# octree-nn/octfusion

Hardware: AMD Instinct MI355X
Metric: denoising-steps/sec (depth-8 octree, batch 8) (higher is better)
Workload: dtype f32 storage, fp16x3 products (fp16 hi + lo operand pairs = 22 significand bits, three fp16 MFMAs per product, fp32 accumulate)

## Files before the change

octfusion_amd/csrc/ofx_dense.hip:

```cpp
#include "ofx_common.h"

__global__ void grid_table_kernel(int mode, int d_out, int B, int32_t pad, int32_t* __restrict__ nbr) {
  const int S = 1 << d_out;
  const int64_t per = (int64_t)S * S * S, total = per * B * 27;
  const int d_in = mode == 0 ? d_out : (mode == 1 ? d_out + 1 : d_out - 1);
  const int Sin = 1 << d_in;
  for (int64_t t = (int64_t)blockIdx.x * blockDim.x + threadIdx.x; t < total; t += (int64_t)gridDim.x * blockDim.x) {
    const int64_t row = t / 27;
    const int tap = (int)(t - row * 27);
    const int64_t b = row / per;
    int x, y, z, bb;
    ofx_key2xyz(row - b * per, x, y, z, bb);
    const int tx = tap / 9 - 1, ty = (tap / 3) % 3 - 1, tz = tap % 3 - 1;
    int ix, iy, iz;
    bool ok;
    if (mode == 0) {
      ix = x + tx; iy = y + ty; iz = z + tz;
      ok = ix >= 0 && iy >= 0 && iz >= 0 && ix < S && iy < S && iz < S;
    } else if (mode == 1) {
      ix = 2 * x + tx; iy = 2 * y + ty; iz = 2 * z + tz;
      ok = ix >= 0 && iy >= 0 && iz >= 0 && ix < Sin && iy < Sin && iz < Sin;
    } else {
      const int fx = x + tx, fy = y + ty, fz = z + tz;
      ok = fx >= 0 && fy >= 0 && fz >= 0 && fx < S && fy < S && fz < S;
      ix = fx >> 1; iy = fy >> 1; iz = fz >> 1;
    }
    nbr[t] = ok ? (int32_t)(b * ((int64_t)Sin * Sin * Sin) + (int64_t)ofx_xyz2morton(ix, iy, iz)) : pad;
  }
}

extern "C" int ofx_grid_conv_table(int mode, int depth_out, int batch_size, int32_t pad, int32_t* nbr27, void* stream) {
  if (mode < 0 || mode > 2 || depth_out < 0 || depth_out > 8 || batch_size < 1 || !nbr27) return OFX_EINVAL;
  if (mode == 2 && depth_out < 1) return OFX_EINVAL;
  const int64_t total = (1ll << (3 * depth_out)) * batch_size * 27;
  grid_table_kernel<<<ofx_grid(total, 256), 256, 0, ofx_stream(stream)>>>(mode, depth_out, batch_size, pad, nbr27);
  OFX_LAUNCH_CHECK();
  return OFX_OK;
}

typedef float f32x16d __attribute__((ext_vector_type(16)));

template <int CH, bool SPLIT>
__global__ void __launch_bounds__(256, 1) attention_mfma_kernel(const float* __restrict__ qkv, int64_t ldq, int T,
                                                                int heads, int ch, float* __restrict__ out,
                                                                int64_t ldo) {
  __shared__ float cmb[4][32][2];
  constexpr int KLD = CH + 4;
  extern __shared__ __attribute__((aligned(16))) float smem[];
  const int Tp = (T + 31) & ~31;
  float* Ks = smem;
  float* Vs = smem + (size_t)Tp * KLD;
  const int bh = blockIdx.x;
  const int b = bh / heads, hd = bh - b * heads;
  const int64_t row0 = (int64_t)b * T;
  const float scale = 1.f / sqrtf(sqrtf((float)ch));
  const int lane = threadIdx.x & 63, wid = threadIdx.x >> 6;
  const int l31 = lane & 31, h = lane >> 5;

  const float* kbase = qkv + row0 * ldq + (int64_t)hd * 3 * ch + ch;
  if ((ch & 3) == 0 && (ldq & 3) == 0 && (((uintptr_t)qkv) & 15) == 0) {
    constexpr int C4 = CH / 4;
    const int total = Tp * C4;
    for (int i0 = threadIdx.x; i0 < total; i0 += 4 * blockDim.x) {
      float4 kq[4], vq[4];
#pragma unroll
      for (int u = 0; u < 4; ++u) {
        const int i = i0 + u * blockDim.x;
        const int s = i / C4, c = (i - s * C4) * 4;
        kq[u] = make_float4(0.f, 0.f, 0.f, 0.f);
        vq[u] = kq[u];
        if (i < total && s < T && c < ch) {
          const float* p = kbase + (int64_t)s * ldq + c;
          kq[u] = *reinterpret_cast<const float4*>(p);
          vq[u] = *reinterpret_cast<const float4*>(p + ch);
        }
      }
#pragma unroll
      for (int u = 0; u < 4; ++u) {
        const int i = i0 + u * blockDim.x;
        if (i >= total) continue;
        const int s = i / C4, c = (i - s * C4) * 4;
        *reinterpret_cast<float4*>(Ks + s * KLD + c) = make_float4(kq[u].x * scale, kq[u].y * scale, kq[u].z * scale, kq[u].w * scale);
        *reinterpret_cast<float4*>(Vs + s * KLD + c) = vq[u];
      }
    }
  } else {
    for (int i = threadIdx.x; i < Tp * CH; i += blockDim.x) {
      const int s = i / CH, c = i - s * CH;
      float kv = 0.f, vv = 0.f;
      if (s < T && c < ch) {
        const float* p = kbase + (int64_t)s * ldq + c;
        kv = p[0] * scale;
        vv = p[ch];
      }
      Ks[s * KLD + c] = kv;
      Vs[s * KLD + c] = vv;
    }
  }
  __syncthreads();

  const int q0 = SPLIT ? blockIdx.y * 32 : blockIdx.y * 128 + wid * 32;
  if (q0 >= T) return;
  const int qi = q0 + l31;
  const bool qok = qi < T;
  float qreg[CH / 2];
  {
    const float* qp = qkv + (row0 + (qok ? qi : T - 1)) * ldq + (int64_t)hd * 3 * ch;
#pragma unroll
    for (int s = 0; s < CH / 2; ++s) {
      const int c = h * (CH / 2) + s;
      qreg[s] = (c < ch) ? qp[c] * scale : 0.f;
    }
  }
  const int ntile = Tp / 32;

  auto score_tile = [&](int kt, f32x16d& st) {
#pragma unroll
    for (int r = 0; r < 16; ++r) st[r] = 0.f;
    const float* kr = Ks + (kt * 32 + l31) * KLD + h * (CH / 2);
#pragma unroll
    for (int s4 = 0; s4 < CH / 8; ++s4) {
      const float4 kv = *reinterpret_cast<const float4*>(kr + s4 * 4);
      st = __builtin_amdgcn_mfma_f32_32x32x2f32(kv.x, qreg[s4 * 4 + 0], st, 0, 0, 0);
      st = __builtin_amdgcn_mfma_f32_32x32x2f32(kv.y, qreg[s4 * 4 + 1], st, 0, 0, 0);
      st = __builtin_amdgcn_mfma_f32_32x32x2f32(kv.z, qreg[s4 * 4 + 2], st, 0, 0, 0);
      st = __builtin_amdgcn_mfma_f32_32x32x2f32(kv.w, qreg[s4 * 4 + 3], st, 0, 0, 0);
    }
    if (kt * 32 + 32 > T) {
#pragma unroll
      for (int r = 0; r < 16; ++r)
        if (kt * 32 + (r & 3) + 8 * (r >> 2) + 4 * h >= T) st[r] = -INFINITY;
    }
  };

  const int kt0 = SPLIT ? (wid * ntile) / 4 : 0, kt1 = SPLIT ? ((wid + 1) * ntile) / 4 : ntile;

  float mx = -INFINITY, den = 0.f;
  for (int kt = kt0; kt < kt1; ++kt) {
    f32x16d st;
    score_tile(kt, st);
    float tm = st[0];
#pragma unroll
    for (int r = 1; r < 16; ++r) tm = fmaxf(tm, st[r]);
    tm = fmaxf(tm, __shfl_xor(tm, 32, 64));
    const float mn = fmaxf(mx, tm);
    float ps = 0.f;
#pragma unroll
    for (int r = 0; r < 16; ++r) ps += __expf(st[r] - mn);
    ps += __shfl_xor(ps, 32, 64);
    den = den * __expf(mx - mn) + ps;
    mx = mn;
  }
  if (SPLIT) {
    if (h == 0) { cmb[wid][l31][0] = mx; cmb[wid][l31][1] = den; }
    __syncthreads();
    float gm = -INFINITY;
#pragma unroll
    for (int w = 0; w < 4; ++w) gm = fmaxf(gm, cmb[w][l31][0]);
    float gd = 0.f;
#pragma unroll
    for (int w = 0; w < 4; ++w) {
      const float mw = cmb[w][l31][0];
      gd += mw == -INFINITY ? 0.f : cmb[w][l31][1] * __expf(mw - gm);
    }
    mx = gm; den = gd;
  }
  const float inv = 1.f / den;

  f32x16d oacc[CH / 32];
#pragma unroll
  for (int j = 0; j < CH / 32; ++j)
#pragma unroll
    for (int r = 0; r < 16; ++r) oacc[j][r] = 0.f;
  for (int kt = kt0; kt < kt1; ++kt) {
    f32x16d st;
    score_tile(kt, st);
#pragma unroll
    for (int r = 0; r < 16; ++r) st[r] = __expf(st[r] - mx) * inv;
    const float* vr = Vs + (kt * 32 + 4 * h) * KLD + l31;
#pragma unroll
    for (int r = 0; r < 16; ++r) {
      const float* vrow = vr + ((r & 3) + 8 * (r >> 2)) * KLD;
#pragma unroll
      for (int j = 0; j < CH / 32; ++j)
        oacc[j] = __builtin_amdgcn_mfma_f32_32x32x2f32(st[r], vrow[j * 32], oacc[j], 0, 0, 0);
    }
  }
  if (SPLIT) {
    __syncthreads();
    float* osum = Ks;
#pragma unroll
    for (int j = 0; j < CH / 32; ++j)
#pragma unroll
      for (int r = 0; r < 16; ++r)
        osum[(wid * 32 + (r & 3) + 8 * (r >> 2) + 4 * h) * CH + j * 32 + l31] = oacc[j][r];
    __syncthreads();
    for (int i = threadIdx.x; i < 32 * CH; i += 256) {
      const int q = i / CH, c = i - q * CH;
      if (q0 + q < T && c < ch)
        out[(row0 + q0 + q) * ldo + (int64_t)hd * ch + c] = (osum[i] + osum[32 * CH + i]) + (osum[64 * CH + i] + osum[96 * CH + i]);
    }
    return;
  }
#pragma unroll
  for (int j = 0; j < CH / 32; ++j) {
    const int c = j * 32 + l31;
    if (c >= ch) continue;
#pragma unroll
    for (int r = 0; r < 16; ++r) {
      const int q = q0 + (r & 3) + 8 * (r >> 2) + 4 * h;
      if (q < T) out[(row0 + q) * ldo + (int64_t)hd * ch + c] = oacc[j][r];
    }
  }
}

static int g_attn_split = 1;
extern "C" int ofx_set_attention_split(int on) { g_attn_split = on ? 1 : 0; return OFX_OK; }

template <int CH>
static int launch_attention(const float* qkv, int64_t ldq, int B, int T, int heads, int ch, float* out, int64_t ldo,
                            hipStream_t st) {
  const int Tp = (T + 31) & ~31;
  const size_t lds = (size_t)2 * Tp * (CH + 4) * sizeof(float);
  if (lds > 160 * 1024 - 2048) return OFX_EINVAL;
  static bool attr_set[OFX_MAX_DEVICES] = {}, attr_set_split[OFX_MAX_DEVICES] = {};
  if (T >= 256 && g_attn_split) {
    if (!ofx_raise_lds_limit(reinterpret_cast<const void*>(&attention_mfma_kernel<CH, true>), 160 * 1024 - 2048, attr_set_split))
      return OFX_ELAUNCH;
    dim3 grid((unsigned)(B * heads), (unsigned)ofx_cdiv(T, 32));
    attention_mfma_kernel<CH, true><<<grid, 256, lds, st>>>(qkv, ldq, T, heads, ch, out, ldo);
    return OFX_OK;
  }
  if (!ofx_raise_lds_limit(reinterpret_cast<const void*>(&attention_mfma_kernel<CH, false>), 160 * 1024 - 2048, attr_set))
    return OFX_ELAUNCH;
  dim3 grid((unsigned)(B * heads), (unsigned)ofx_cdiv(T, 128));
  attention_mfma_kernel<CH, false><<<grid, 256, lds, st>>>(qkv, ldq, T, heads, ch, out, ldo);
  return OFX_OK;
}

extern "C" int ofx_attention(const float* qkv, int64_t ldq, int batch_size, int T, int heads, int ch, float* out,
                             int64_t ldo, void* stream) {
  if (!qkv || !out || batch_size < 1 || T < 1 || heads < 1 || ch < 1 || ch > 128 || ldq < 3 * (int64_t)heads * ch ||
      ldo < (int64_t)heads * ch)
    return OFX_EINVAL;
  hipStream_t st = ofx_stream(stream);
  int rc;
  if (ch <= 32) rc = launch_attention<32>(qkv, ldq, batch_size, T, heads, ch, out, ldo, st);
  else if (ch <= 64) rc = launch_attention<64>(qkv, ldq, batch_size, T, heads, ch, out, ldo, st);
  else rc = launch_attention<128>(qkv, ldq, batch_size, T, heads, ch, out, ldo, st);
  if (rc) return rc;
  OFX_LAUNCH_CHECK();
  return OFX_OK;
}


__device__ __forceinline__ float score_rounded(float a, float sc) {
#pragma clang fp contract(off)
  return a * sc;
}
__device__ __forceinline__ float wave_sum(float v) {
#pragma unroll
  for (int o = 32; o > 0; o >>= 1) v += __shfl_xor(v, o);
  return v;
}
__device__ __forceinline__ float wave_max(float v) {
#pragma unroll
  for (int o = 32; o > 0; o >>= 1) v = fmaxf(v, __shfl_xor(v, o));
  return v;
}

__global__ void __launch_bounds__(256) attention_bwd_q_kernel(const float* __restrict__ qkv, int64_t ldq,
                                                              const float* __restrict__ dout, int64_t ldo, int T,
                                                              int heads, int ch, float* __restrict__ rowstat,
                                                              float* __restrict__ dqkv, int64_t ldd) {
  extern __shared__ float lds[];
  const int lane = threadIdx.x & 63, wid = threadIdx.x >> 6;
  const int bh = blockIdx.y, b = bh / heads, hd = bh - b * heads;
  const int i = blockIdx.x * 4 + wid;
  if (i >= T) return;
  float* ds = lds + wid * T;
  const float sc = rsqrtf((float)ch);
  const int64_t row0 = (int64_t)b * T;
  const float* qi = qkv + (row0 + i) * ldq + (int64_t)hd * 3 * ch;
  const float* gi = dout + (row0 + i) * ldo + (int64_t)hd * ch;
  const float* kb = qkv + row0 * ldq + (int64_t)hd * 3 * ch + ch;
  const float* vb = kb + ch;
  const bool vec = (ch & 3) == 0 && (ldq & 3) == 0 && (ldo & 3) == 0 && ((((uintptr_t)qkv) | ((uintptr_t)dout)) & 15) == 0;
  float s[8], dp[8];
  float m = -3.0e38f;
#pragma unroll
  for (int t = 0; t < 8; ++t) {
    const int j = lane + 64 * t;
    s[t] = -3.0e38f; dp[t] = 0.f;
    if (j < T) {
      float a = 0.f, d = 0.f;
      const float* kj = kb + (int64_t)j * ldq;
      const float* vj = vb + (int64_t)j * ldq;
      if (vec) {
        for (int c = 0; c < ch; c += 4) {
          const float4 q4 = *reinterpret_cast<const float4*>(qi + c), g4 = *reinterpret_cast<const float4*>(gi + c);
          const float4 k4 = *reinterpret_cast<const float4*>(kj + c), v4 = *reinterpret_cast<const float4*>(vj + c);
          a += q4.x * k4.x + q4.y * k4.y + q4.z * k4.z + q4.w * k4.w;
          d += g4.x * v4.x + g4.y * v4.y + g4.z * v4.z + g4.w * v4.w;
        }
      } else {
        for (int c = 0; c < ch; ++c) { a += qi[c] * kj[c]; d += gi[c] * vj[c]; }
      }
      s[t] = score_rounded(a, sc); dp[t] = d;
      m = fmaxf(m, s[t]);
    }
  }
  m = wave_max(m);
  float l = 0.f;
#pragma unroll
  for (int t = 0; t < 8; ++t) { const int j = lane + 64 * t; if (j < T) { s[t] = __expf(s[t] - m); l += s[t]; } }
  l = wave_sum(l);
  const float inv = 1.f / l;
  float D = 0.f;
#pragma unroll
  for (int t = 0; t < 8; ++t) { const int j = lane + 64 * t; if (j < T) { s[t] *= inv; D += s[t] * dp[t]; } }
  D = wave_sum(D);
#pragma unroll
  for (int t = 0; t < 8; ++t) { const int j = lane + 64 * t; if (j < T) ds[j] = s[t] * (dp[t] - D); }
  if (lane == 0) {
    float* rs = rowstat + ((int64_t)bh * T + i) * 3;
    rs[0] = m; rs[1] = inv; rs[2] = D;
  }
  __builtin_amdgcn_wave_barrier();
  for (int c = lane; c < ch; c += 64) {
    float a = 0.f;
    for (int j = 0; j < T; ++j) a += ds[j] * kb[(int64_t)j * ldq + c];
    dqkv[(row0 + i) * ldd + (int64_t)hd * 3 * ch + c] = a * sc;
  }
}

__global__ void __launch_bounds__(256) attention_bwd_kv_kernel(const float* __restrict__ qkv, int64_t ldq,
                                                               const float* __restrict__ dout, int64_t ldo, int T,
                                                               int heads, int ch, const float* __restrict__ rowstat,
                                                               float* __restrict__ dqkv, int64_t ldd) {
  extern __shared__ float lds[];
  const int lane = threadIdx.x & 63, wid = threadIdx.x >> 6;
  const int bh = blockIdx.y, b = bh / heads, hd = bh - b * heads;
  const int j = blockIdx.x * 4 + wid;
  if (j >= T) return;
  float* pc = lds + wid * 2 * T;
  float* dc = pc + T;
  const float sc = rsqrtf((float)ch);
  const int64_t row0 = (int64_t)b * T;
  const float* qb = qkv + row0 * ldq + (int64_t)hd * 3 * ch;
  const float* kj = qb + (int64_t)j * ldq + ch;
  const float* vj = kj + ch;
  const float* gb = dout + row0 * ldo + (int64_t)hd * ch;
  const float* rs = rowstat + (int64_t)bh * T * 3;
  const bool vec = (ch & 3) == 0 && (ldq & 3) == 0 && (ldo & 3) == 0 && ((((uintptr_t)qkv) | ((uintptr_t)dout)) & 15) == 0;
  for (int i = lane; i < T; i += 64) {
    float a = 0.f, d = 0.f;
    const float* qr = qb + (int64_t)i * ldq;
    const float* gr = gb + (int64_t)i * ldo;
    if (vec) {
      for (int c = 0; c < ch; c += 4) {
        const float4 q4 = *reinterpret_cast<const float4*>(qr + c), g4 = *reinterpret_cast<const float4*>(gr + c);
        const float4 k4 = *reinterpret_cast<const float4*>(kj + c), v4 = *reinterpret_cast<const float4*>(vj + c);
        a += q4.x * k4.x + q4.y * k4.y + q4.z * k4.z + q4.w * k4.w;
        d += g4.x * v4.x + g4.y * v4.y + g4.z * v4.z + g4.w * v4.w;
      }
    } else {
      for (int c = 0; c < ch; ++c) { a += qr[c] * kj[c]; d += gr[c] * vj[c]; }
    }
    const float p = __expf(score_rounded(a, sc) - rs[i * 3]) * rs[i * 3 + 1];
    pc[i] = p;
    dc[i] = p * (d - rs[i * 3 + 2]);
  }
  __builtin_amdgcn_wave_barrier();
  for (int c = lane; c < ch; c += 64) {
    float dk = 0.f, dv = 0.f;
    for (int i = 0; i < T; ++i) { dk += dc[i] * qb[(int64_t)i * ldq + c]; dv += pc[i] * gb[(int64_t)i * ldo + c]; }
    float* o = dqkv + (row0 + j) * ldd + (int64_t)hd * 3 * ch;
    o[ch + c] = dk * sc;
    o[2 * ch + c] = dv;
  }
}

extern "C" int ofx_attention_bwd(const float* qkv, int64_t ldq, const float* dout, int64_t ldo, int batch_size, int T,
                                 int heads, int ch, float* rowstat, float* dqkv, int64_t ldd, void* stream) {
  if (!qkv || !dout || !rowstat || !dqkv || batch_size < 1 || T < 1 || T > 512 || heads < 1 || ch < 1 ||
      ldq < 3 * (int64_t)heads * ch || ldd < 3 * (int64_t)heads * ch || ldo < (int64_t)heads * ch)
    return OFX_EINVAL;
  hipStream_t st = ofx_stream(stream);
  const dim3 grid((unsigned)((T + 3) / 4), (unsigned)(batch_size * heads));
  attention_bwd_q_kernel<<<grid, 256, 4 * T * sizeof(float), st>>>(qkv, ldq, dout, ldo, T, heads, ch, rowstat, dqkv, ldd);
  attention_bwd_kv_kernel<<<grid, 256, 8 * T * sizeof(float), st>>>(qkv, ldq, dout, ldo, T, heads, ch, rowstat, dqkv, ldd);
  OFX_LAUNCH_CHECK();
  return OFX_OK;
}
```

Before: 121.9.

## Add direct-from-global attention kernel with register-cached scores for small head dims

For head dims up to 64, adds a new attention kernel that loads K and V rows straight from global memory into registers with double-buffered prefetch, instead of staging the whole K/V sequence in LDS. Score tiles are kept in registers between the softmax-statistics pass and the PV pass, so the QK^T MFMAs are not recomputed. Key tiles are split across up to four waves, whose results are combined through shared memory. Shared softmax helpers are factored out of the existing kernel. The number of register-cached tiles per wave is capped by a template constant, so longer sequences than that cap would not be fully covered, and the larger register footprint may limit occupancy.

```diff
diff --git a/octfusion_amd/csrc/ofx_dense.hip b/octfusion_amd/csrc/ofx_dense.hip
--- a/octfusion_amd/csrc/ofx_dense.hip
+++ b/octfusion_amd/csrc/ofx_dense.hip
@@ -40,6 +40,39 @@
 
 typedef float f32x16d __attribute__((ext_vector_type(16)));
 
+__device__ __forceinline__ void attn_mask_tile(f32x16d& st, int kt, int h, int T) {
+  if (kt * 32 + 32 > T) {
+#pragma unroll
+    for (int r = 0; r < 16; ++r)
+      if (kt * 32 + (r & 3) + 8 * (r >> 2) + 4 * h >= T) st[r] = -INFINITY;
+  }
+}
+__device__ __forceinline__ void attn_stats_tile(const f32x16d& st, float& mx, float& den) {
+  float tm = st[0];
+#pragma unroll
+  for (int r = 1; r < 16; ++r) tm = fmaxf(tm, st[r]);
+  tm = fmaxf(tm, __shfl_xor(tm, 32, 64));
+  const float mn = fmaxf(mx, tm);
+  float ps = 0.f;
+#pragma unroll
+  for (int r = 0; r < 16; ++r) ps += __expf(st[r] - mn);
+  ps += __shfl_xor(ps, 32, 64);
+  den = den * __expf(mx - mn) + ps;
+  mx = mn;
+}
+__device__ __forceinline__ void attn_combine_stats(float (*cmb)[32][2], int nw, int wid, int l31, int h, float& mx, float& den) {
+  if (h == 0) { cmb[wid][l31][0] = mx; cmb[wid][l31][1] = den; }
+  __syncthreads();
+  float gm = -INFINITY;
+  for (int w = 0; w < nw; ++w) gm = fmaxf(gm, cmb[w][l31][0]);
+  float gd = 0.f;
+  for (int w = 0; w < nw; ++w) {
+    const float mw = cmb[w][l31][0];
+    gd += mw == -INFINITY ? 0.f : cmb[w][l31][1] * __expf(mw - gm);
+  }
+  mx = gm; den = gd;
+}
+
 template <int CH, bool SPLIT>
 __global__ void __launch_bounds__(256, 1) attention_mfma_kernel(const float* __restrict__ qkv, int64_t ldq, int T,
                                                                 int heads, int ch, float* __restrict__ out,
@@ -126,11 +159,7 @@
       st = __builtin_amdgcn_mfma_f32_32x32x2f32(kv.z, qreg[s4 * 4 + 2], st, 0, 0, 0);
       st = __builtin_amdgcn_mfma_f32_32x32x2f32(kv.w, qreg[s4 * 4 + 3], st, 0, 0, 0);
     }
-    if (kt * 32 + 32 > T) {
-#pragma unroll
-      for (int r = 0; r < 16; ++r)
-        if (kt * 32 + (r & 3) + 8 * (r >> 2) + 4 * h >= T) st[r] = -INFINITY;
-    }
+    attn_mask_tile(st, kt, h, T);
   };
 
   const int kt0 = SPLIT ? (wid * ntile) / 4 : 0, kt1 = SPLIT ? ((wid + 1) * ntile) / 4 : ntile;
@@ -139,32 +168,9 @@
   for (int kt = kt0; kt < kt1; ++kt) {
     f32x16d st;
     score_tile(kt, st);
-    float tm = st[0];
-#pragma unroll
-    for (int r = 1; r < 16; ++r) tm = fmaxf(tm, st[r]);
-    tm = fmaxf(tm, __shfl_xor(tm, 32, 64));
-    const float mn = fmaxf(mx, tm);
-    float ps = 0.f;
-#pragma unroll
-    for (int r = 0; r < 16; ++r) ps += __expf(st[r] - mn);
-    ps += __shfl_xor(ps, 32, 64);
-    den = den * __expf(mx - mn) + ps;
-    mx = mn;
-  }
-  if (SPLIT) {
-    if (h == 0) { cmb[wid][l31][0] = mx; cmb[wid][l31][1] = den; }
-    __syncthreads();
-    float gm = -INFINITY;
-#pragma unroll
-    for (int w = 0; w < 4; ++w) gm = fmaxf(gm, cmb[w][l31][0]);
-    float gd = 0.f;
-#pragma unroll
-    for (int w = 0; w < 4; ++w) {
-      const float mw = cmb[w][l31][0];
-      gd += mw == -INFINITY ? 0.f : cmb[w][l31][1] * __expf(mw - gm);
-    }
-    mx = gm; den = gd;
-  }
+    attn_stats_tile(st, mx, den);
+  }
+  if (SPLIT) attn_combine_stats(cmb, 4, wid, l31, h, mx, den);
   const float inv = 1.f / den;
 
   f32x16d oacc[CH / 32];
@@ -214,8 +220,157 @@
   }
 }
 
+__device__ __forceinline__ float attn_ld(const float* base, uint32_t byte_off) {
+  return *reinterpret_cast<const float*>(reinterpret_cast<const char*>(base) + byte_off);
+}
+template <int CH, bool VEC>
+__device__ __forceinline__ void attn_load_k(const float* base, uint32_t krow, int c0, int ch, float4 (&kf)[CH / 8]) {
+  if (VEC) {
+#pragma unroll
+    for (int s4 = 0; s4 < CH / 8; ++s4)
+      kf[s4] = *reinterpret_cast<const float4*>(reinterpret_cast<const char*>(base) + (krow + 4u * min(c0 + s4 * 4, ch - 4)));
+  } else {
+#pragma unroll
+    for (int s4 = 0; s4 < CH / 8; ++s4) {
+      const int c = c0 + s4 * 4;
+      kf[s4] = make_float4(attn_ld(base, krow + 4u * min(c, ch - 1)), attn_ld(base, krow + 4u * min(c + 1, ch - 1)),
+                           attn_ld(base, krow + 4u * min(c + 2, ch - 1)), attn_ld(base, krow + 4u * min(c + 3, ch - 1)));
+    }
+  }
+}
+
+template <int CH, bool VEC, int NT>
+__global__ void __launch_bounds__(256, 2) attention_direct_kernel(const float* __restrict__ qkv, int64_t ldq, int T, int heads,
+                                                                  int ch, float* __restrict__ out, int64_t ldo) {
+  __shared__ float cmb[4][32][2];
+  __shared__ float osum[4 * 32 * CH];
+  const int bh = blockIdx.x;
+  const int b = bh / heads, hd = bh - b * heads;
+  const int64_t row0 = (int64_t)b * T;
+  const float scale = 1.f / sqrtf(sqrtf((float)ch));
+  const int lane = threadIdx.x & 63, wid = threadIdx.x >> 6, nw = blockDim.x >> 6;
+  const int l31 = lane & 31, h = lane >> 5;
+  const float* base = qkv + row0 * ldq + (int64_t)hd * 3 * ch;
+  const uint32_t pitch = 4u * (uint32_t)ldq;
+  const int c0 = h * (CH / 2);
+  const int ntile = (T + 31) >> 5;
+  const int kt0 = (wid * ntile) / nw, nt = ((wid + 1) * ntile) / nw - kt0;
+  auto k_row = [&](int kt) { return (uint32_t)min(kt * 32 + l31, T - 1) * pitch + 4u * ch; };
+
+  float4 kf[2][CH / 8];
+  attn_load_k<CH, VEC>(base, k_row(kt0), c0, ch, kf[0]);
+
+  const int q0 = blockIdx.y * 32;
+  const int qi = q0 + l31;
+  float qreg[CH / 2];
+  {
+    float4 qf[CH / 8];
+    attn_load_k<CH, VEC>(base, (uint32_t)min(qi, T - 1) * pitch, c0, ch, qf);
+#pragma unroll
+    for (int s4 = 0; s4 < CH / 8; ++s4) {
+      const int c = c0 + s4 * 4;
+      qreg[s4 * 4 + 0] = c + 0 < ch ? qf[s4].x * scale : 0.f;
+      qreg[s4 * 4 + 1] = c + 1 < ch ? qf[s4].y * scale : 0.f;
+      qreg[s4 * 4 + 2] = c + 2 < ch ? qf[s4].z * scale : 0.f;
+      qreg[s4 * 4 + 3] = c + 3 < ch ? qf[s4].w * scale : 0.f;
+    }
+  }
+  uint32_t vcol[CH / 32];
+#pragma unroll
+  for (int j = 0; j < CH / 32; ++j) vcol[j] = 4u * (2 * ch + min(j * 32 + l31, ch - 1));
+  auto load_v = [&](int kt, float (&vf)[16][CH / 32]) {
+#pragma unroll
+    for (int r = 0; r < 16; ++r) {
+      const uint32_t vrow = (uint32_t)min(kt * 32 + 4 * h + (r & 3) + 8 * (r >> 2), T - 1) * pitch;
+#pragma unroll
+      for (int j = 0; j < CH / 32; ++j) vf[r][j] = attn_ld(base, vrow + vcol[j]);
+    }
+  };
+
+  float vf[2][16][CH / 32];
+  load_v(kt0, vf[0]);
+
+  f32x16d sc[NT];
+  float mx = -INFINITY, den = 0.f;
+#pragma unroll
+  for (int i = 0; i < NT; ++i) {
+    if (i > 0 && i >= nt) break;
+    if (i + 1 < NT && i + 1 < nt) attn_load_k<CH, VEC>(base, k_row(kt0 + i + 1), c0, ch, kf[(i + 1) & 1]);
+    __builtin_amdgcn_sched_barrier(0);
+    const int kt = kt0 + i;
+    f32x16d st;
+#pragma unroll
+    for (int r = 0; r < 16; ++r) st[r] = 0.f;
+    const bool kok = kt * 32 + l31 < T;
+#pragma unroll
+    for (int s4 = 0; s4 < CH / 8; ++s4) {
+      const int c = c0 + s4 * 4;
+      const float4 kv = kf[i & 1][s4];
+      st = __builtin_amdgcn_mfma_f32_32x32x2f32(kok && c + 0 < ch ? kv.x * scale : 0.f, qreg[s4 * 4 + 0], st, 0, 0, 0);
+      st = __builtin_amdgcn_mfma_f32_32x32x2f32(kok && c + 1 < ch ? kv.y * scale : 0.f, qreg[s4 * 4 + 1], st, 0, 0, 0);
+      st = __builtin_amdgcn_mfma_f32_32x32x2f32(kok && c + 2 < ch ? kv.z * scale : 0.f, qreg[s4 * 4 + 2], st, 0, 0, 0);
+      st = __builtin_amdgcn_mfma_f32_32x32x2f32(kok && c + 3 < ch ? kv.w * scale : 0.f, qreg[s4 * 4 + 3], st, 0, 0, 0);
+    }
+    attn_mask_tile(st, kt, h, T);
+    attn_stats_tile(st, mx, den);
+    sc[i] = st;
+  }
+  if (nw > 1) attn_combine_stats(cmb, nw, wid, l31, h, mx, den);
+  const float inv = 1.f / den;
+
+  f32x16d oacc[CH / 32];
+#pragma unroll
+  for (int j = 0; j < CH / 32; ++j)
+#pragma unroll
+    for (int r = 0; r < 16; ++r) oacc[j][r] = 0.f;
+#pragma unroll
+  for (int i = 0; i < NT; ++i) {
+    if (i > 0 && i >= nt) break;
+    if (i + 1 < NT && i + 1 < nt) load_v(kt0 + i + 1, vf[(i + 1) & 1]);
+    __builtin_amdgcn_sched_barrier(0);
+    const int kt = kt0 + i;
+    f32x16d st = sc[i];
+#pragma unroll
+    for (int r = 0; r < 16; ++r) st[r] = __expf(st[r] - mx) * inv;
+#pragma unroll
+    for (int r = 0; r < 16; ++r) {
+      const bool vok = kt * 32 + 4 * h + (r & 3) + 8 * (r >> 2) < T;
+#pragma unroll
+      for (int j = 0; j < CH / 32; ++j)
+        oacc[j] = __builtin_amdgcn_mfma_f32_32x32x2f32(st[r], vok && j * 32 + l31 < ch ? vf[i & 1][r][j] : 0.f, oacc[j], 0, 0, 0);
+    }
+  }
+  if (nw == 1) {
+#pragma unroll
+    for (int j = 0; j < CH / 32; ++j) {
+      const int c = j * 32 + l31;
+      if (c >= ch) continue;
+#pragma unroll
+      for (int r = 0; r < 16; ++r) {
+        const int q = q0 + (r & 3) + 8 * (r >> 2) + 4 * h;
+        if (q < T) out[(row0 + q) * ldo + (int64_t)hd * ch + c] = oacc[j][r];
+      }
+    }
+    return;
+  }
+#pragma unroll
+  for (int j = 0; j < CH / 32; ++j)
+#pragma unroll
+    for (int r = 0; r < 16; ++r)
+      osum[(wid * 32 + (r & 3) + 8 * (r >> 2) + 4 * h) * CH + j * 32 + l31] = oacc[j][r];
+  __syncthreads();
+  for (int i = threadIdx.x; i < 32 * CH; i += blockDim.x) {
+    const int q = i / CH, c = i - q * CH;
+    if (q0 + q < T && c < ch) {
+      float o = osum[i] + osum[32 * CH + i];
+      if (nw > 2) o += nw > 3 ? osum[64 * CH + i] + osum[96 * CH + i] : osum[64 * CH + i];
+      out[(row0 + q0 + q) * ldo + (int64_t)hd * ch + c] = o;
+    }
+  }
+}
+
 static int g_attn_split = 1;
-extern "C" int ofx_set_attention_split(int on) { g_attn_split = on ? 1 : 0; return OFX_OK; }
+extern "C" int ofx_set_attention_split(int on) { g_attn_split = on == 2 ? 2 : (on ? 1 : 0); return OFX_OK; }
 
 template <int CH>
 static int launch_attention(const float* qkv, int64_t ldq, int B, int T, int heads, int ch, float* out, int64_t ldo,
@@ -223,6 +378,23 @@
   const int Tp = (T + 31) & ~31;
   const size_t lds = (size_t)2 * Tp * (CH + 4) * sizeof(float);
   if (lds > 160 * 1024 - 2048) return OFX_EINVAL;
+  if constexpr (CH <= 64) {
+    if (g_attn_split == 1 && (int64_t)T * ldq < (1ll << 30)) {
+      const int ntile = Tp / 32;
+      dim3 grid((unsigned)(B * heads), (unsigned)ntile);
+      const dim3 block(64 * (ntile < 4 ? ntile : 4));
+      const bool vec = (ch & 3) == 0 && (ldq & 3) == 0 && (((uintptr_t)qkv) & 15) == 0;
+      constexpr int NTMAX = CH == 32 ? 5 : 3;
+      if (ntile <= 4) {
+        if (vec) attention_direct_kernel<CH, true, 1><<<grid, block, 0, st>>>(qkv, ldq, T, heads, ch, out, ldo);
+        else attention_direct_kernel<CH, false, 1><<<grid, block, 0, st>>>(qkv, ldq, T, heads, ch, out, ldo);
+      } else {
+        if (vec) attention_direct_kernel<CH, true, NTMAX><<<grid, block, 0, st>>>(qkv, ldq, T, heads, ch, out, ldo);
+        else attention_direct_kernel<CH, false, NTMAX><<<grid, block, 0, st>>>(qkv, ldq, T, heads, ch, out, ldo);
+      }
+      return OFX_OK;
+    }
+  }
   static bool attr_set[OFX_MAX_DEVICES] = {}, attr_set_split[OFX_MAX_DEVICES] = {};
   if (T >= 256 && g_attn_split) {
     if (!ofx_raise_lds_limit(reinterpret_cast<const void*>(&attention_mfma_kernel<CH, true>), 160 * 1024 - 2048, attr_set_split))
```

New measurement: 122.8 (median of 6 runs). No clear change (+0.8%).
